# sourmash-bio/sourmash

Measured on AMD Instinct MI355X. Metric: Gbase/s sketched (k=31, scaled=1000), higher is better.
Workload: dtype u64; 1 GPU; C2: sketch synthetic random DNA resident in HBM as ASCII, per GPU 1000 records of 10000000 bases (10000000000 bases, 10000001000 bytes with their separators), k=31 scaled=1000 seed=42; one step = k-mer kernel + radix sort + unique; records_per_gpu=1000, record_len=10000000, bases_per_gpu=10000000000, bytes_per_gpu=10000001000, ksize=31, scaled=1000, unique_hashes_rank0=9998668, unique_hashes_job=9998668, collectives=none (the exchange runs with --full)

## Files before the change

### sourmash_amd/csrc/kmer_core.hpp

```cpp
#pragma once
#include "murmur3.hpp"
#include <utility>

namespace smg {

SMG_HD uint32_t perm_b32(uint32_t hi, uint32_t lo, uint32_t sel) {
#if defined(__HIP_DEVICE_COMPILE__)
    return __builtin_amdgcn_perm(hi, lo, sel);
#else
    const uint64_t v = ((uint64_t)hi << 32) | lo;
    uint32_t r = 0;
    for (int i = 0; i < 4; ++i) {
        const uint32_t s = (sel >> (8 * i)) & 0xff;
        uint32_t b;
        if (s < 8) b = (uint32_t)(v >> (8 * s)) & 0xff;
        else if (s == 0x0c) b = 0;
        else b = 0xff;
        r |= b << (8 * i);
    }
    return r;
#endif
}

SMG_HD uint32_t alignbyte_b32(uint32_t hi, uint32_t lo, uint32_t n) {
#if defined(__HIP_DEVICE_COMPILE__)
    return __builtin_amdgcn_alignbyte(hi, lo, n);
#else
    return (uint32_t)((((uint64_t)hi << 32) | lo) >> (8 * n));
#endif
}

SMG_HD bool any_lane(bool p) {
#if defined(__HIP_DEVICE_COMPILE__)
    return __builtin_amdgcn_ballot_w64(p) != 0ull;
#else
    return p;
#endif
}

SMG_HD uint32_t bitselect(uint32_t mask, uint32_t b, uint32_t c) {
#if defined(__HIP_DEVICE_COMPILE__)
    return __builtin_amdgcn_bitop3_b32(mask, b, c, 0xCA);
#else
    return (mask & b) | (~mask & c);
#endif
}

SMG_HD uint32_t opaque(uint32_t x) {
#if defined(__HIP_DEVICE_COMPILE__)
    asm volatile("" : "+v"(x));
#endif
    return x;
}

SMG_HD uint32_t bswap32(uint32_t x) { return perm_b32(0u, x, 0x00010203u); }

constexpr uint32_t LUT_SELF = 'A' | ('C' << 8) | ('T' << 16) | ((uint32_t)'G' << 24);
constexpr uint32_t LUT_COMP = 'T' | ('G' << 8) | ('A' << 16) | ((uint32_t)'C' << 24);

template <int K, int P>
struct LaneGeom {
    static constexpr int NBYTES = P + K - 1;
    static constexpr int NW = (NBYTES + 3) / 4;
    static constexpr int NWK = (K + 3) / 4;
    static constexpr int NCH = (K + 7) / 8;
    static constexpr uint32_t LAST_MASK = (K % 4) ? ((1u << (8 * (K % 4))) - 1u) : 0xffffffffu;
};

constexpr uint32_t rev_sel(int a) {
    return (uint32_t)(a + 3) | ((uint32_t)(a + 2) << 8) | ((uint32_t)(a + 1) << 16) | ((uint32_t)a << 24);
}
constexpr uint32_t rev_sel_partial(int a, int nb) {
    uint32_t s = 0;
    for (int i = 0; i < 4; ++i) {
        const uint32_t b = (i < nb) ? (uint32_t)(a + nb - 1 - i) : 0x0cu;
        s |= b << (8 * i);
    }
    return s;
}

template <int K, int P, int O>
struct PosOps {
    using G = LaneGeom<K, P>;

    template <int D>
    static SMG_HD uint32_t fwd(const uint32_t* U) {
        constexpr int q = (O >> 2) + D, a = O & 3;
        uint32_t v;
        if constexpr (a == 0) v = U[q];
        else if constexpr (q + 1 < G::NW) v = alignbyte_b32(U[q + 1], U[q], a);
        else v = U[q] >> (8 * a);
        if constexpr (D == G::NWK - 1) v &= G::LAST_MASK;
        return v;
    }

    template <int D>
    static SMG_HD uint32_t rev(const uint32_t* C) {
        constexpr int nb = (K - 4 * D) >= 4 ? 4 : (K - 4 * D);
        constexpr int s = O + K - 4 * D - nb;
        constexpr int q = s >> 2, a = s & 3;
        constexpr uint32_t sel = (nb == 4) ? rev_sel(a) : rev_sel_partial(a, nb);
        if constexpr (q + 1 < G::NW) return perm_b32(C[q + 1], C[q], sel);
        else return perm_b32(0u, C[q], sel);
    }

    template <int CH>
    static SMG_HD uint64_t be_chunk(const uint32_t* W) {
        uint64_t v = (uint64_t)bswap32(W[2 * CH]) << 32;
        if constexpr (2 * CH + 1 < G::NWK) v |= bswap32(W[2 * CH + 1]);
        return v;
    }

    template <int CH>
    static SMG_HD uint64_t be_chunk_opaque(const uint32_t* W) {
        uint64_t v = (uint64_t)bswap32(opaque(W[2 * CH])) << 32;
        if constexpr (2 * CH + 1 < G::NWK) v |= bswap32(opaque(W[2 * CH + 1]));
        return v;
    }

    template <int CH>
    static SMG_HD void tie_break(const uint32_t* F, const uint32_t* R, bool& tie, bool& gt) {
        if constexpr (CH < G::NCH) {
            const uint64_t bf = be_chunk_opaque<CH>(F), br = be_chunk_opaque<CH>(R);
            gt = gt || (tie && bf > br);
            tie = tie && (bf == br);
            tie_break<CH + 1>(F, R, tie, gt);
        }
    }

    template <int... D>
    static SMG_HD void build(const uint32_t* U, const uint32_t* C, uint32_t* F, uint32_t* R,
                             std::integer_sequence<int, D...>) {
        ((F[D] = fwd<D>(U)), ...);
        ((R[D] = rev<D>(C)), ...);
    }

    template <bool PLAIN = false>
    static SMG_HD Mmh3Open hash_open(const uint32_t* U, const uint32_t* C, uint64_t seed) {
        uint32_t F[G::NWK], R[G::NWK];
        build(U, C, F, R, std::make_integer_sequence<int, G::NWK>{});
        const uint64_t bf = be_chunk<0>(F), br = be_chunk<0>(R);
        bool gt = bf > br;
        bool tie = bf == br;
        if (G::NCH > 1 && any_lane(tie)) tie_break<1>(F, R, tie, gt);
        uint32_t W[G::NWK];
        const uint32_t m = gt ? 0xffffffffu : 0u;
#pragma unroll
        for (int d = 0; d < G::NWK; ++d) W[d] = bitselect(m, R[d], F[d]);
        return mmh3_open_words<K, PLAIN>(W, seed);
    }
};

SMG_HD uint32_t nonzero_bytes4(uint32_t x) {
    uint32_t t = x | (x >> 4);
    t |= t >> 2;
    t |= t >> 1;
    t &= 0x01010101u;
    return (t * 0x01020408u) >> 24 & 0xfu;
}

SMG_HD uint32_t early_limit(uint64_t thr) {
    const uint32_t thr_hi = (uint32_t)(thr >> 32);
    return thr_hi >= 0xfffffffdu ? 0xffffffffu : thr_hi + 2u;
}
SMG_HD bool early_may_keep(Mmh3Open open, uint32_t lim) { return (uint32_t)(mmh3_close_hi_sum(open) + 1u) <= lim; }

template <int K, int P, bool EARLY, bool PLAIN, bool STAGED, class Emit, int... O>
SMG_HD void process_window(const uint32_t* raw, const uint32_t* comp, bool dirty, uint64_t seed, uint64_t thr, Emit&& emit,
                           std::integer_sequence<int, O...>) {
    using G = LaneGeom<K, P>;
    const uint32_t lim = early_limit(thr);
    uint32_t Ubuf[STAGED ? 1 : G::NW], Cbuf[STAGED ? 1 : G::NW];
    const uint32_t* U = STAGED ? raw : Ubuf;
    const uint32_t* C = STAGED ? comp : Cbuf;
    uint32_t anybad = 0;
    if constexpr (!STAGED) {
#pragma unroll
        for (int i = 0; i < G::NW; ++i) {
            const uint32_t u = raw[i] & 0xdfdfdfdfu;
            const uint32_t code = (u >> 1) & 0x03030303u;
            Ubuf[i] = u;
            Cbuf[i] = perm_b32(0u, LUT_COMP, code);
            uint32_t bad = perm_b32(0u, LUT_SELF, code) ^ u;
            if (i == G::NW - 1 && (G::NBYTES % 4) != 0)
                bad &= (1u << (8 * (G::NBYTES % 4))) - 1u;
            anybad |= bad;
        }
    }
    uint64_t badlo = 0, badhi = 0, badtop = 0;
    if (!STAGED || dirty) {
        if constexpr (STAGED) {
#pragma unroll
            for (int i = 0; i < G::NW; ++i) {
                const uint32_t u = U[i];
                uint32_t bad = perm_b32(0u, LUT_SELF, (u >> 1) & 0x03030303u) ^ u;
                if (i == G::NW - 1 && (G::NBYTES % 4) != 0)
                    bad &= (1u << (8 * (G::NBYTES % 4))) - 1u;
                anybad |= bad;
            }
        }
        if (anybad != 0) {
#pragma unroll
            for (int i = 0; i < G::NW; ++i) {
                const uint32_t u = U[i];
                const uint32_t code = (u >> 1) & 0x03030303u;
                uint32_t bad = perm_b32(0u, LUT_SELF, code) ^ u;
                if (i == G::NW - 1 && (G::NBYTES % 4) != 0) bad &= (1u << (8 * (G::NBYTES % 4))) - 1u;
                const uint64_t nib = nonzero_bytes4(bad);
                if (4 * i < 64) badlo |= nib << (4 * i);
                else if (4 * i < 128) badhi |= nib << (4 * i - 64);
                else badtop |= nib << (4 * i - 128);
            }
        }
    }
    static_assert(G::NBYTES <= 192 && K <= 128 && P <= 64, "window too long for the 192-bit validity mask");
    (
        [&] {
            const Mmh3Open open = PosOps<K, P, O>::template hash_open<PLAIN>(U, C, seed);
            if constexpr (EARLY) {
                if (!any_lane(early_may_keep(open, lim))) return;
            }
            const uint64_t h = mmh3_close<PLAIN>(open);
            bool ok = (h - 1) < thr;
            if (anybad != 0) {
                uint64_t lo, hi;
                if constexpr (O == 0) { lo = badlo; hi = badhi; }
                else { lo = (badlo >> O) | (badhi << (64 - O)); hi = (badhi >> O) | (badtop << (64 - O)); }
                const uint64_t mlo = K >= 64 ? ~0ull : ((1ull << K) - 1);
                const uint64_t mhi = K >= 128 ? ~0ull : K > 64 ? ((1ull << (K - 64)) - 1) : 0;
                if ((lo & mlo) | (hi & mhi)) ok = false;
            }
            if (ok) emit(O, h);
        }(),
        ...);
}

template <int K, int P, bool EARLY = true, bool PLAIN = false, class Emit>
SMG_HD void process_lane(const uint32_t* raw, uint64_t seed, uint64_t thr, Emit&& emit) {
    process_window<K, P, EARLY, PLAIN, false>(raw, nullptr, false, seed, thr, static_cast<Emit&&>(emit),
                                              std::make_integer_sequence<int, P>{});
}
template <int K, int P, bool EARLY = true, bool PLAIN = false, class Emit>
SMG_HD void process_lane_staged(const uint32_t* U, const uint32_t* C, bool dirty, uint64_t seed, uint64_t thr, Emit&& emit) {
    process_window<K, P, EARLY, PLAIN, true>(U, C, dirty, seed, thr, static_cast<Emit&&>(emit), std::make_integer_sequence<int, P>{});
}


template <int K, int P, int BLOCK, int R = 1>
struct TileGeom {
    using G = LaneGeom<K, P>;
    static constexpr int WINDOW = BLOCK * P;
    static constexpr int TILE = R * WINDOW;
    static constexpr int LANE_RD = ((G::NW + 3) / 4) * 4;
    static constexpr int chunks(int rounds) { return ((rounds * BLOCK - 1) * (P / 4) + LANE_RD + 3) / 4; }
    static constexpr int IN_DW = (R * BLOCK - 1) * (P / 4) + LANE_RD;
    static constexpr int IN_CHUNKS = chunks(R);
};

SMG_HD uint32_t sk_tile_rounds(uint64_t thr, uint32_t r_max, uint32_t window, uint32_t cap) {
    if (r_max <= 1) return 1;
    const uint64_t positions = (uint64_t)r_max * window;
    const uint64_t expected = (positions * (thr >> 32)) >> 32;
    return expected + 1 > cap / 4 ? 1u : r_max;
}

SMG_HD uint64_t tile_first(uint32_t workgroup) { return workgroup; }
SMG_HD uint64_t tile_from_ticket(uint32_t grid, uint64_t ticket) { return (uint64_t)grid + ticket; }
SMG_HD bool tile_end(uint64_t tile, uint64_t n_tiles) { return tile >= n_tiles; }

SMG_HD void load_chunk(const uint8_t* seq, uint64_t off, uint64_t len, uint32_t skip, uint32_t* w) {
    w[0] = w[1] = w[2] = w[3] = 0;
    if (off + 16 <= len) {
#if defined(__HIP_DEVICE_COMPILE__)
        const uint4 v = *reinterpret_cast<const uint4*>(seq + off);
        w[0] = v.x; w[1] = v.y; w[2] = v.z; w[3] = v.w;
#else
        for (int b = 0; b < 16; ++b) w[b >> 2] |= (uint32_t)seq[off + b] << (8 * (b & 3));
#endif
    } else if (off < len) {
        for (uint64_t b = off; b < len; ++b) w[(b - off) >> 2] |= (uint32_t)seq[b] << (8 * ((b - off) & 3));
    }
    if (off == 0 && skip) {
        for (uint32_t b = 0; b < skip; ++b) w[b >> 2] &= ~(0xffu << (8 * (b & 3)));
    }
}

SMG_HD uint32_t stage_chunk(uint32_t* w, uint32_t* c) {
    uint32_t anybad = 0;
#pragma unroll
    for (int j = 0; j < 4; ++j) {
        const uint32_t u = w[j] & 0xdfdfdfdfu;
        const uint32_t code = (u >> 1) & 0x03030303u;
        w[j] = u;
        c[j] = perm_b32(0u, LUT_COMP, code);
        anybad |= perm_b32(0u, LUT_SELF, code) ^ u;
    }
    return anybad;
}

SMG_HD void store_chunk(uint32_t* dst, const uint32_t* w) {
#if defined(__HIP_DEVICE_COMPILE__)
    *reinterpret_cast<uint4*>(dst) = make_uint4(w[0], w[1], w[2], w[3]);
#else
    dst[0] = w[0]; dst[1] = w[1]; dst[2] = w[2]; dst[3] = w[3];
#endif
}

template <int IN_CHUNKS, bool STAGED, int BLOCK>
SMG_HD void stage_tile(const uint8_t* seq, uint64_t base, uint64_t len, uint32_t skip, uint32_t* s_in, uint32_t* s_comp,
                       unsigned int* s_dirty, int n_chunks = IN_CHUNKS) {
#if defined(__HIP_DEVICE_COMPILE__)
    const int first = threadIdx.x, step = BLOCK;
#else
    const int first = 0, step = 1;
#endif
    for (int c = first; c < n_chunks; c += step) {
        uint32_t w[4];
        load_chunk(seq, base + (uint64_t)c * 16, len, skip, w);
        if constexpr (STAGED) {
            uint32_t cw[4];
            if (stage_chunk(w, cw)) *s_dirty = 1;
            store_chunk(&s_comp[c * 4], cw);
        }
        store_chunk(&s_in[c * 4], w);
    }
}

template <int LANE_RD, int P>
SMG_HD void read_window(const uint32_t* s, int tid, uint32_t* out) {
    static_assert(P % 4 == 0 && LANE_RD % 4 == 0, "lane runs must start dword aligned");
    const uint32_t* p = &s[tid * (P / 4)];
#pragma unroll
    for (int i = 0; i < LANE_RD / 4; ++i) {
#if defined(__HIP_DEVICE_COMPILE__)
        if constexpr ((P / 4) % 4 == 0) {
            const uint4 v = reinterpret_cast<const uint4*>(p)[i];
            out[4 * i] = v.x; out[4 * i + 1] = v.y; out[4 * i + 2] = v.z; out[4 * i + 3] = v.w;
            continue;
        }
#endif
        out[4 * i] = p[4 * i]; out[4 * i + 1] = p[4 * i + 1]; out[4 * i + 2] = p[4 * i + 2]; out[4 * i + 3] = p[4 * i + 3];
    }
}

#if defined(__HIPCC__)
template <int CAP, int BLOCK, int NV = 1>
struct LdsSink {
    uint64_t* s_val[NV];
    unsigned int* s_cnt;
    unsigned long long* s_base;
    uint64_t* out[NV];
    unsigned long long* out_count;
    uint64_t out_cap;

    template <class... V>
    __device__ __forceinline__ void append(V... v) const {
        static_assert(sizeof...(V) == NV, "one value per array");
        const uint64_t e[NV] = {(uint64_t)v...};
        const unsigned int idx = atomicAdd(s_cnt, 1u);
        if (idx < (unsigned)CAP) {
#pragma unroll
            for (int j = 0; j < NV; ++j) s_val[j][idx] = e[j];
        } else {
            const unsigned long long g = atomicAdd(out_count, 1ull);
            if (g < out_cap) {
#pragma unroll
                for (int j = 0; j < NV; ++j) out[j][g] = e[j];
            }
        }
    }
    __device__ __forceinline__ void flush(unsigned int at_least) const {
        const unsigned int cnt = *s_cnt;
        if (cnt < at_least) return;
        const unsigned int n = cnt < (unsigned)CAP ? cnt : (unsigned)CAP;
        if (threadIdx.x == 0) *s_base = atomicAdd(out_count, (unsigned long long)n);
        __syncthreads();
        const unsigned long long b = *s_base;
        for (unsigned int i = threadIdx.x; i < n; i += BLOCK) {
            if (b + i < out_cap) {
#pragma unroll
                for (int j = 0; j < NV; ++j) out[j][b + i] = s_val[j][i];
            }
        }
        __syncthreads();
        if (threadIdx.x == 0) *s_cnt = 0;
    }
};
#endif

}
```

### sourmash_amd/csrc/sketch_kernel.hpp

```cpp
#pragma once
#include <hip/hip_runtime.h>
#include <stdint.h>
#include <utility>
#include "kmer_core.hpp"
#include "tile_launch.hpp"
#include "arena.hpp"

namespace smg {

constexpr int SK_BLOCK = 256;
constexpr int SK_FAST_MAX_K = 88;
constexpr int SK_OUT_CAP = 2048;

constexpr bool sk_plain_mul(int k, bool dense) {
    if (dense) return k == 1 || k == 5 || k == 8 || k == 25 || k == 28 || k == 81 || k == 82 || k == 84;
    return k == 50 || k == 51;
}
constexpr bool sk_staged(int k) { return k > 11 && k != 18 && k != 20 && k != 30; }
#ifndef SMG_SK_R_MAX
#define SMG_SK_R_MAX 3
#endif
constexpr int SK_R_MAX = SMG_SK_R_MAX;
static_assert(SK_R_MAX >= 1 && SK_R_MAX <= 3, "four rounds do not fit four workgroups per CU");
constexpr bool sk_one_round(int k) { return k <= 17; }
constexpr int sk_rounds_max(int k, bool dense) { return !dense && sk_staged(k) && !sk_one_round(k) ? SK_R_MAX : 1; }
constexpr int sk_out_cap(int r_max) { return r_max >= 3 ? SK_OUT_CAP / 2 : SK_OUT_CAP; }
#ifdef SMG_SK_STATIC_WALK
constexpr bool sk_handout(int) { return false; }
#else
constexpr bool sk_handout(int) { return true; }
#endif
#ifdef SMG_SK_GRID_PER_CU
constexpr unsigned sk_grid_per_cu(int, bool) { return SMG_SK_GRID_PER_CU; }
#else
constexpr unsigned sk_grid_per_cu(int r_max, bool handout) { return handout ? 0 : r_max > 1 ? 32 : 8; }
#endif

template <int K, int P, bool DENSE>
__global__ __launch_bounds__(SK_BLOCK) void sketch_dna_kernel(
    const uint8_t* __restrict__ seq, uint64_t len, uint64_t seed, uint64_t thr,
    uint64_t* __restrict__ out, unsigned long long* __restrict__ out_count, uint64_t out_cap,
    uint64_t n_tiles, uint32_t skip, uint32_t rounds, unsigned long long* __restrict__ tile_counter) {
    constexpr int R_MAX = sk_rounds_max(K, DENSE), OUT_CAP = sk_out_cap(R_MAX);
    using T = TileGeom<K, P, SK_BLOCK, R_MAX>;
    constexpr int WINDOW = T::WINDOW, LANE_RD = T::LANE_RD, IN_CHUNKS = T::IN_CHUNKS;
    constexpr bool STAGED = !DENSE && sk_staged(K);
    static_assert(R_MAX == 1 || STAGED, "only the staged form walks several rounds");
    const uint32_t n_rounds = R_MAX > 1 ? rounds : 1u;

    __shared__ __attribute__((aligned(16))) uint32_t s_in[IN_CHUNKS * 4];
    __shared__ __attribute__((aligned(16))) uint32_t s_comp[STAGED ? IN_CHUNKS * 4 : 4];
    __shared__ unsigned int s_dirty;
    __shared__ uint64_t s_out[OUT_CAP];
    __shared__ unsigned int s_cnt;
    __shared__ unsigned long long s_base;
    __shared__ unsigned long long s_next;
    const bool handout = !DENSE && sk_handout(K) && tile_counter != nullptr;
    const LdsSink<OUT_CAP, SK_BLOCK> sink{{s_out}, &s_cnt, &s_base, {out}, out_count, out_cap};

    const int tid = threadIdx.x;
    if (tid == 0) s_cnt = 0;

    uint64_t tile = tile_first(blockIdx.x);
    while (!tile_end(tile, n_tiles)) {
        const uint64_t base = tile * ((uint64_t)n_rounds * WINDOW);
        if constexpr (STAGED) {
            if (tid == 0) s_dirty = 0;
        }
        __syncthreads();
        if constexpr (STAGED) {
            if constexpr (R_MAX > 1) stage_tile<IN_CHUNKS, true, SK_BLOCK>(seq, base, len, skip, s_in, s_comp, &s_dirty, T::chunks((int)n_rounds));
            else stage_tile<IN_CHUNKS, true, SK_BLOCK>(seq, base, len, skip, s_in, s_comp, &s_dirty);
        } else {
            for (int c = tid; c < IN_CHUNKS; c += SK_BLOCK) {
                const uint64_t off = base + (uint64_t)c * 16;
                uint4 v = make_uint4(0, 0, 0, 0);
                if (off + 16 <= len) {
                    v = *reinterpret_cast<const uint4*>(seq + off);
                } else if (off < len) {
                    uint32_t w[4] = {0, 0, 0, 0};
                    for (uint64_t b = off; b < len; ++b) w[(b - off) >> 2] |= (uint32_t)seq[b] << (8 * ((b - off) & 3));
                    v = make_uint4(w[0], w[1], w[2], w[3]);
                }
                if (off == 0 && skip) {
                    uint32_t w[4] = {v.x, v.y, v.z, v.w};
                    for (uint32_t b = 0; b < skip; ++b) w[b >> 2] &= ~(0xffu << (8 * (b & 3)));
                    v = make_uint4(w[0], w[1], w[2], w[3]);
                }
                *reinterpret_cast<uint4*>(&s_in[c * 4]) = v;
            }
        }
        __syncthreads();
        if constexpr (!DENSE && sk_handout(K)) {
            if (handout && tid == 0) s_next = tile_from_ticket(gridDim.x, atomicAdd(tile_counter, 1ull));
        }
        uint32_t raw[LANE_RD];
        if constexpr (R_MAX == 1) read_window<LANE_RD, P>(s_in, tid, raw);
        auto emit = [&](int o, uint64_t h) {
            if constexpr (DENSE) {
                const uint64_t pos = base + (uint64_t)tid * P + (uint64_t)o - skip;
                if (pos < out_cap) out[pos] = h;
            } else {
                sink.append(h);
            }
        };
        if constexpr (STAGED) {
            static_assert(!STAGED || P == 16, "the staged form reads whole 16-byte groups");
            uint32_t comp[LANE_RD];
            if constexpr (R_MAX == 1) {
                read_window<LANE_RD, P>(s_comp, tid, comp);
                const bool dirty = __builtin_amdgcn_readfirstlane(s_dirty) != 0;
                process_lane_staged<K, P, true, sk_plain_mul(K, false)>(raw, comp, dirty, seed, thr, emit);
            } else {
                const bool dirty = __builtin_amdgcn_readfirstlane(s_dirty) != 0;
#pragma unroll 1
                for (uint32_t r = 0; r < n_rounds; ++r) {
                    read_window<LANE_RD, P>(s_in, tid + (int)r * SK_BLOCK, raw);
                    read_window<LANE_RD, P>(s_comp, tid + (int)r * SK_BLOCK, comp);
                    process_lane_staged<K, P, true, sk_plain_mul(K, false)>(raw, comp, dirty, seed, thr, emit);
                }
            }
        } else {
            process_lane<K, P, !DENSE, sk_plain_mul(K, DENSE)>(raw, seed, thr, emit);
        }
        if constexpr (DENSE) { tile += gridDim.x; continue; }
        __syncthreads();
        if (handout) {
            const unsigned long long next = s_next;
            tile = ((uint64_t)(uint32_t)__builtin_amdgcn_readfirstlane((int)(uint32_t)(next >> 32)) << 32) |
                   (uint32_t)__builtin_amdgcn_readfirstlane((int)(uint32_t)next);
        } else {
            tile += gridDim.x;
        }
        sink.flush(OUT_CAP / 2);
    }
    if constexpr (DENSE) return;
    __syncthreads();
    sink.flush(1);
}

typedef hipError_t (*sketch_launch_fn)(const uint8_t*, uint64_t, uint64_t, uint64_t, uint64_t*, unsigned long long*, uint64_t, uint32_t, hipStream_t);
template <int K, bool DENSE>
unsigned sk_resident_grid() {
    static const unsigned resident = [] {
        int per_cu = 0, dev = 0, cus = 0;
        if (hipOccupancyMaxActiveBlocksPerMultiprocessor(&per_cu, (const void*)sketch_dna_kernel<K, 16, DENSE>, SK_BLOCK, 0) != hipSuccess ||
            hipGetDevice(&dev) != hipSuccess || hipDeviceGetAttribute(&cus, hipDeviceAttributeMultiprocessorCount, dev) != hipSuccess ||
            per_cu < 1 || cus < 1) {
            (void)hipGetLastError();
            return 2048u;
        }
        return (unsigned)per_cu * (unsigned)cus;
    }();
    return resident;
}
template <bool DENSE>
struct SketchLaunch {
    using fn = sketch_launch_fn;
    static constexpr int KMAX = SK_FAST_MAX_K;
    template <int K>
    static hipError_t launch(const uint8_t* d_seq, uint64_t len, uint64_t seed, uint64_t thr, uint64_t* d_out,
                             unsigned long long* d_count, uint64_t cap, uint32_t grid, hipStream_t stream) {
        constexpr uint32_t WINDOW = (uint32_t)SK_BLOCK * 16, R_MAX = (uint32_t)sk_rounds_max(K, DENSE);
        const uint32_t rounds = sk_tile_rounds(thr, R_MAX, WINDOW, (uint32_t)sk_out_cap((int)R_MAX));
        const TileSpan t = align_to_tiles(d_seq, len, (uint64_t)rounds * WINDOW);
        if (t.n_tiles == 0) return hipSuccess;
        constexpr unsigned per_cu = sk_grid_per_cu((int)R_MAX, !DENSE && sk_handout(K));
        unsigned g;
        if (grid && !DENSE) {
            g = grid;
        } else if constexpr (per_cu == 0) {
            const unsigned resident = sk_resident_grid<K, DENSE>();
            g = (unsigned)(t.n_tiles < resident ? t.n_tiles : resident);
        } else {
            g = sk_grid(t.n_tiles, per_cu);
        }
        ArenaBuf counter;
        if constexpr (!DENSE && sk_handout(K)) {
            if (t.n_tiles > g) {
                hipError_t e = counter.get(8, stream);
                if (e == hipSuccess) e = hipMemsetAsync(counter.p, 0, 8, stream);
                if (e != hipSuccess) return e;
            }
        }
        hipLaunchKernelGGL((sketch_dna_kernel<K, 16, DENSE>), dim3(g), dim3(SK_BLOCK), 0, stream,
                           t.seq, t.len, seed, thr, d_out, d_count, cap, t.n_tiles, t.skip, rounds, counter.as<unsigned long long>());
        return hipGetLastError();
    }
};

}
```

Before: 376.4 Gbase/s.

## Process 32 positions per lane in staged kernel and defer last-word key mask

Doubles the k-mer positions each lane handles in the staged sketch path (except at some k values), which cuts the rounds per tile and resizes the output buffer to match. The window overlap loads and per-lane setup are spread over more k-mers. The mask on the last partial dword of the canonical key now runs once after choosing forward or reverse, and the reverse path uses full 4-byte permutes. The risks are register pressure and lower occupancy from the larger per-lane window and the longer unrolled position loop.

```diff
diff --git a/sourmash_amd/csrc/kmer_core.hpp b/sourmash_amd/csrc/kmer_core.hpp
--- a/sourmash_amd/csrc/kmer_core.hpp
+++ b/sourmash_amd/csrc/kmer_core.hpp
@@ -65,6 +65,7 @@
     static constexpr int NWK = (K + 3) / 4;
     static constexpr int NCH = (K + 7) / 8;
     static constexpr uint32_t LAST_MASK = (K % 4) ? ((1u << (8 * (K % 4))) - 1u) : 0xffffffffu;
+    static constexpr bool LATE_MASK_OK = (K % 4) != 0 && NWK > 2;
 };
 
 constexpr uint32_t rev_sel(int a) {
@@ -79,9 +80,10 @@
     return s;
 }
 
-template <int K, int P, int O>
+template <int K, int P, int O, bool LATE = false>
 struct PosOps {
     using G = LaneGeom<K, P>;
+    static constexpr bool LATE_MASK = LATE && G::LATE_MASK_OK;
 
     template <int D>
     static SMG_HD uint32_t fwd(const uint32_t* U) {
@@ -90,13 +92,14 @@
         if constexpr (a == 0) v = U[q];
         else if constexpr (q + 1 < G::NW) v = alignbyte_b32(U[q + 1], U[q], a);
         else v = U[q] >> (8 * a);
-        if constexpr (D == G::NWK - 1) v &= G::LAST_MASK;
+        if constexpr (D == G::NWK - 1 && !LATE_MASK) v &= G::LAST_MASK;
         return v;
     }
 
     template <int D>
     static SMG_HD uint32_t rev(const uint32_t* C) {
-        constexpr int nb = (K - 4 * D) >= 4 ? 4 : (K - 4 * D);
+        constexpr int nbk = (K - 4 * D) >= 4 ? 4 : (K - 4 * D);
+        constexpr int nb = (LATE_MASK && O + K - 4 * D - 4 >= 0) ? 4 : nbk;
         constexpr int s = O + K - 4 * D - nb;
         constexpr int q = s >> 2, a = s & 3;
         constexpr uint32_t sel = (nb == 4) ? rev_sel(a) : rev_sel_partial(a, nb);
@@ -111,10 +114,16 @@
         return v;
     }
 
+    template <int D>
+    static SMG_HD uint32_t key_dword_opaque(const uint32_t* W) {
+        const uint32_t v = opaque(W[D]);
+        if constexpr (D == G::NWK - 1 && LATE_MASK) return v & G::LAST_MASK;
+        else return v;
+    }
     template <int CH>
     static SMG_HD uint64_t be_chunk_opaque(const uint32_t* W) {
-        uint64_t v = (uint64_t)bswap32(opaque(W[2 * CH])) << 32;
-        if constexpr (2 * CH + 1 < G::NWK) v |= bswap32(opaque(W[2 * CH + 1]));
+        uint64_t v = (uint64_t)bswap32(key_dword_opaque<2 * CH>(W)) << 32;
+        if constexpr (2 * CH + 1 < G::NWK) v |= bswap32(key_dword_opaque<2 * CH + 1>(W));
         return v;
     }
 
@@ -147,6 +156,7 @@
         const uint32_t m = gt ? 0xffffffffu : 0u;
 #pragma unroll
         for (int d = 0; d < G::NWK; ++d) W[d] = bitselect(m, R[d], F[d]);
+        if constexpr (LATE_MASK) W[G::NWK - 1] &= G::LAST_MASK;
         return mmh3_open_words<K, PLAIN>(W, seed);
     }
 };
@@ -165,7 +175,7 @@
 }
 SMG_HD bool early_may_keep(Mmh3Open open, uint32_t lim) { return (uint32_t)(mmh3_close_hi_sum(open) + 1u) <= lim; }
 
-template <int K, int P, bool EARLY, bool PLAIN, bool STAGED, class Emit, int... O>
+template <int K, int P, bool EARLY, bool PLAIN, bool STAGED, bool LATE, class Emit, int... O>
 SMG_HD void process_window(const uint32_t* raw, const uint32_t* comp, bool dirty, uint64_t seed, uint64_t thr, Emit&& emit,
                            std::integer_sequence<int, O...>) {
     using G = LaneGeom<K, P>;
@@ -216,7 +226,7 @@
     static_assert(G::NBYTES <= 192 && K <= 128 && P <= 64, "window too long for the 192-bit validity mask");
     (
         [&] {
-            const Mmh3Open open = PosOps<K, P, O>::template hash_open<PLAIN>(U, C, seed);
+            const Mmh3Open open = PosOps<K, P, O, LATE>::template hash_open<PLAIN>(U, C, seed);
             if constexpr (EARLY) {
                 if (!any_lane(early_may_keep(open, lim))) return;
             }
@@ -237,12 +247,12 @@
 
 template <int K, int P, bool EARLY = true, bool PLAIN = false, class Emit>
 SMG_HD void process_lane(const uint32_t* raw, uint64_t seed, uint64_t thr, Emit&& emit) {
-    process_window<K, P, EARLY, PLAIN, false>(raw, nullptr, false, seed, thr, static_cast<Emit&&>(emit),
+    process_window<K, P, EARLY, PLAIN, false, false>(raw, nullptr, false, seed, thr, static_cast<Emit&&>(emit),
                                               std::make_integer_sequence<int, P>{});
 }
-template <int K, int P, bool EARLY = true, bool PLAIN = false, class Emit>
+template <int K, int P, bool EARLY = true, bool PLAIN = false, bool LATE = false, class Emit>
 SMG_HD void process_lane_staged(const uint32_t* U, const uint32_t* C, bool dirty, uint64_t seed, uint64_t thr, Emit&& emit) {
-    process_window<K, P, EARLY, PLAIN, true>(U, C, dirty, seed, thr, static_cast<Emit&&>(emit), std::make_integer_sequence<int, P>{});
+    process_window<K, P, EARLY, PLAIN, true, LATE>(U, C, dirty, seed, thr, static_cast<Emit&&>(emit), std::make_integer_sequence<int, P>{});
 }
 
 
diff --git a/sourmash_amd/csrc/sketch_kernel.hpp b/sourmash_amd/csrc/sketch_kernel.hpp
--- a/sourmash_amd/csrc/sketch_kernel.hpp
+++ b/sourmash_amd/csrc/sketch_kernel.hpp
@@ -22,9 +22,27 @@
 #endif
 constexpr int SK_R_MAX = SMG_SK_R_MAX;
 static_assert(SK_R_MAX >= 1 && SK_R_MAX <= 3, "four rounds do not fit four workgroups per CU");
+constexpr bool sk_late_mask(int k) { return sk_staged(k) && k != 13; }
 constexpr bool sk_one_round(int k) { return k <= 17; }
-constexpr int sk_rounds_max(int k, bool dense) { return !dense && sk_staged(k) && !sk_one_round(k) ? SK_R_MAX : 1; }
-constexpr int sk_out_cap(int r_max) { return r_max >= 3 ? SK_OUT_CAP / 2 : SK_OUT_CAP; }
+constexpr bool sk_lane16_only(int k) { return (k >= 35 && k <= 40) || (k >= 53 && k <= 56); }
+#ifndef SMG_SK_LANE_POSITIONS
+#define SMG_SK_LANE_POSITIONS 32
+#endif
+constexpr int sk_lane_positions(int k, bool dense) {
+    return !dense && sk_staged(k) && !sk_one_round(k) && !sk_lane16_only(k) ? SMG_SK_LANE_POSITIONS : 16;
+}
+#ifndef SMG_SK_LANE32_R_MAX
+#define SMG_SK_LANE32_R_MAX 2
+#endif
+static_assert(SMG_SK_LANE32_R_MAX >= 1 && SMG_SK_LANE32_R_MAX <= 2, "three rounds of 8,192 positions do not fit four workgroups per CU");
+constexpr int sk_rounds_max(int k, bool dense) {
+    if (dense || !sk_staged(k) || sk_one_round(k)) return 1;
+    return sk_lane_positions(k, dense) == 32 ? SMG_SK_LANE32_R_MAX : SK_R_MAX;
+}
+constexpr int sk_out_cap(int r_max, int lane_positions = 16) {
+    const int tile = r_max * SK_BLOCK * lane_positions;
+    return tile >= 16384 ? SK_OUT_CAP / 4 : tile >= 12288 ? SK_OUT_CAP / 2 : SK_OUT_CAP;
+}
 #ifdef SMG_SK_STATIC_WALK
 constexpr bool sk_handout(int) { return false; }
 #else
@@ -41,8 +59,10 @@
     const uint8_t* __restrict__ seq, uint64_t len, uint64_t seed, uint64_t thr,
     uint64_t* __restrict__ out, unsigned long long* __restrict__ out_count, uint64_t out_cap,
     uint64_t n_tiles, uint32_t skip, uint32_t rounds, unsigned long long* __restrict__ tile_counter) {
-    constexpr int R_MAX = sk_rounds_max(K, DENSE), OUT_CAP = sk_out_cap(R_MAX);
-    using T = TileGeom<K, P, SK_BLOCK, R_MAX>;
+    static_assert(P == 16, "the kernel's name; the lane's positions are LP");
+    constexpr int LP = sk_lane_positions(K, DENSE);
+    constexpr int R_MAX = sk_rounds_max(K, DENSE), OUT_CAP = sk_out_cap(R_MAX, LP);
+    using T = TileGeom<K, LP, SK_BLOCK, R_MAX>;
     constexpr int WINDOW = T::WINDOW, LANE_RD = T::LANE_RD, IN_CHUNKS = T::IN_CHUNKS;
     constexpr bool STAGED = !DENSE && sk_staged(K);
     static_assert(R_MAX == 1 || STAGED, "only the staged form walks several rounds");
@@ -95,33 +115,33 @@
             if (handout && tid == 0) s_next = tile_from_ticket(gridDim.x, atomicAdd(tile_counter, 1ull));
         }
         uint32_t raw[LANE_RD];
-        if constexpr (R_MAX == 1) read_window<LANE_RD, P>(s_in, tid, raw);
+        if constexpr (R_MAX == 1) read_window<LANE_RD, LP>(s_in, tid, raw);
         auto emit = [&](int o, uint64_t h) {
             if constexpr (DENSE) {
-                const uint64_t pos = base + (uint64_t)tid * P + (uint64_t)o - skip;
+                const uint64_t pos = base + (uint64_t)tid * LP + (uint64_t)o - skip;
                 if (pos < out_cap) out[pos] = h;
             } else {
                 sink.append(h);
             }
         };
         if constexpr (STAGED) {
-            static_assert(!STAGED || P == 16, "the staged form reads whole 16-byte groups");
+            static_assert(!STAGED || LP == 16 || LP == 32, "the staged form reads whole 16-byte groups");
             uint32_t comp[LANE_RD];
             if constexpr (R_MAX == 1) {
-                read_window<LANE_RD, P>(s_comp, tid, comp);
+                read_window<LANE_RD, LP>(s_comp, tid, comp);
                 const bool dirty = __builtin_amdgcn_readfirstlane(s_dirty) != 0;
-                process_lane_staged<K, P, true, sk_plain_mul(K, false)>(raw, comp, dirty, seed, thr, emit);
+                process_lane_staged<K, LP, true, sk_plain_mul(K, false), sk_late_mask(K)>(raw, comp, dirty, seed, thr, emit);
             } else {
                 const bool dirty = __builtin_amdgcn_readfirstlane(s_dirty) != 0;
 #pragma unroll 1
                 for (uint32_t r = 0; r < n_rounds; ++r) {
-                    read_window<LANE_RD, P>(s_in, tid + (int)r * SK_BLOCK, raw);
-                    read_window<LANE_RD, P>(s_comp, tid + (int)r * SK_BLOCK, comp);
-                    process_lane_staged<K, P, true, sk_plain_mul(K, false)>(raw, comp, dirty, seed, thr, emit);
+                    read_window<LANE_RD, LP>(s_in, tid + (int)r * SK_BLOCK, raw);
+                    read_window<LANE_RD, LP>(s_comp, tid + (int)r * SK_BLOCK, comp);
+                    process_lane_staged<K, LP, true, sk_plain_mul(K, false), sk_late_mask(K)>(raw, comp, dirty, seed, thr, emit);
                 }
             }
         } else {
-            process_lane<K, P, !DENSE, sk_plain_mul(K, DENSE)>(raw, seed, thr, emit);
+            process_lane<K, LP, !DENSE, sk_plain_mul(K, DENSE)>(raw, seed, thr, emit);
         }
         if constexpr (DENSE) { tile += gridDim.x; continue; }
         __syncthreads();
@@ -161,8 +181,9 @@
     template <int K>
     static hipError_t launch(const uint8_t* d_seq, uint64_t len, uint64_t seed, uint64_t thr, uint64_t* d_out,
                              unsigned long long* d_count, uint64_t cap, uint32_t grid, hipStream_t stream) {
-        constexpr uint32_t WINDOW = (uint32_t)SK_BLOCK * 16, R_MAX = (uint32_t)sk_rounds_max(K, DENSE);
-        const uint32_t rounds = sk_tile_rounds(thr, R_MAX, WINDOW, (uint32_t)sk_out_cap((int)R_MAX));
+        constexpr uint32_t LP = (uint32_t)sk_lane_positions(K, DENSE), WINDOW = (uint32_t)SK_BLOCK * LP;
+        constexpr uint32_t R_MAX = (uint32_t)sk_rounds_max(K, DENSE);
+        const uint32_t rounds = sk_tile_rounds(thr, R_MAX, WINDOW, (uint32_t)sk_out_cap((int)R_MAX, (int)LP));
         const TileSpan t = align_to_tiles(d_seq, len, (uint64_t)rounds * WINDOW);
         if (t.n_tiles == 0) return hipSuccess;
         constexpr unsigned per_cu = sk_grid_per_cu((int)R_MAX, !DENSE && sk_handout(K));
```

Result: faster. 385.6 Gbase/s (median of 6 runs) (+2.5%).
